# gonewest818/raytrace-clj

Measured on AMD Instinct MI355X. Metric: Msamples/sec (nx*ny*ns), higher is better.
Workload: dtype f64; 1 GPU; C3: 1920x1080x256spp Shirley cover scene n=50 (10001 spheres), depth 50, thin-lens camera, seeded counter RNG; accel=bvh; 8x8 tiles dealt round-robin to 1 GPU(s); nx=1920, ny=1080, ns=256, spheres=10001, depth=50, accel=bvh, accel_ran=bvh, frames_in_flight=1, launch_form=one GPU

## Files before the change

include/rtmi.h:

```cpp
#ifndef RTMI_H
#define RTMI_H

#include <stdint.h>

#ifdef __cplusplus
extern "C" {
#endif

#define RTMI_OK 0
#define RTMI_E_ARG (-1)
#define RTMI_E_DEVICE (-2)
#define RTMI_E_UNSUPPORTED (-3)
#define RTMI_E_NOMEM (-4)
#define RTMI_E_STATE (-5)

enum { RTMI_PRIM_SPHERE = 0, RTMI_PRIM_UVSPHERE = 1, RTMI_PRIM_MOVING = 2,
       RTMI_PRIM_RECT_XY = 3, RTMI_PRIM_RECT_XZ = 4, RTMI_PRIM_RECT_YZ = 5, RTMI_PRIM_TRIANGLE = 6,
       RTMI_PRIM_MEDIUM = 7, RTMI_PRIM_BOUNDARY = 16 };
enum { RTMI_XFORM_TRANSLATE = 0, RTMI_XFORM_ROTATE_Y = 1 };
enum { RTMI_MAT_LAMBERTIAN = 0, RTMI_MAT_METAL = 1, RTMI_MAT_DIELECTRIC = 2, RTMI_MAT_DIFFUSE_LIGHT = 3,
       RTMI_MAT_ISOTROPIC = 4  };
enum { RTMI_TEX_CONSTANT = 0, RTMI_TEX_UVGRADIENT = 1, RTMI_TEX_CHECKER = 2,
       RTMI_TEX_PERLIN_NOISE = 3, RTMI_TEX_PERLIN_TURB = 4, RTMI_TEX_MARBLE = 5, RTMI_TEX_FLIP_U = 6, RTMI_TEX_FLIP_V = 7,
       RTMI_TEX_IMAGE = 8 };
// ... 162 lines not shown
uint64_t rtmi_sample_key(uint64_t seed, uint64_t pixel, uint64_t sample);
int rtmi_probe_arith(rtmi_ctx *ctx, int32_t n, const double *abc, double *out);
#define RTMI_PROBE_MATH_SLOTS 12
int rtmi_probe_math2(rtmi_ctx *ctx, int32_t n, const double *abc, double tmin, double tmax, int32_t n_slots, double *out);
int rtmi_probe_math(rtmi_ctx *ctx, int32_t n, const double *abc, double tmin, double tmax, double *out);

int rtmi_test_build_tree(int32_t n, const double *geom, const double *cam, int32_t threads, uint64_t *out_hash, int32_t *out_info, double *out_ms);
int rtmi_test_camera_fixed(int32_t cam_kind, const double *cam);
int rtmi_test_half_outward(double x, int32_t up);
int rtmi_test_pack_materials(int32_t n_prims, const int32_t *prim_kind, const double *prim_geom, const int32_t *prim_mat,
                             int32_t n_mats, const int32_t *mat_kind, const int32_t *mat_tex, const double *mat_param,
                             int32_t n_tex, const int32_t *tex_kind, const double *tex_param, const int32_t *tex_child,
                             int32_t cam_kind, const double *cam, const int32_t *prim_flip, const int32_t *prim_xform,
                             int32_t n_xforms, const int32_t *xform_kind, const double *xform_param, int32_t through_creation,
                             uint64_t *out_hash, int32_t *out_facts);
int rtmi_test_pack_geometry(int32_t n_prims, const int32_t *prim_kind, const double *prim_geom, const int32_t *prim_mat,
                            int32_t n_mats, const int32_t *mat_kind, const int32_t *mat_tex, const double *mat_param,
                            int32_t n_tex, const int32_t *tex_kind, const double *tex_param, const int32_t *tex_child,
                            int32_t cam_kind, const double *cam, const int32_t *prim_flip, const int32_t *prim_xform,
                            int32_t n_xforms, const int32_t *xform_kind, const double *xform_param, int32_t through_creation, uint64_t *out_hash);
int rtmi_test_refit(int32_t n_prims, const int32_t *prim_kind, const int32_t *prim_flip, const int32_t *prim_xform, int32_t n_xforms, const int32_t *xform_kind,
                    int32_t cam_kind, const double *cam, int32_t n_steps, const double *geoms, const double *xforms,
                    void *out_nodes, int64_t capacity, int64_t *out_bytes, int32_t *out_info, int32_t *out_big,
                    int32_t *out_cells, int64_t cells_capacity, void *out_leaf_box);
int rtmi_test_refit_half(double x, int32_t up);
int rtmi_test_scene_nodes(rtmi_scene *scene, void *buf, int64_t capacity, int64_t *out_bytes);

#ifdef __cplusplus
}
#endif
// ... 2 lines not shown
```

raytrace_clj_amd/_ffi.py:

```python
import ctypes as C
import os

import numpy as np

try:
    import torch
except ImportError:
    torch = None

_HERE = os.path.dirname(os.path.abspath(__file__))
LIB_PATH = os.environ.get("RTMI_LIB") or os.path.join(_HERE, "lib", "librtmi.so")

SYMBOLS = [
    "rtmi_last_error", "rtmi_backend_name", "rtmi_version", "rtmi_init", "rtmi_shutdown", "rtmi_set_option",
    "rtmi_device_info", "rtmi_scene_create", "rtmi_scene_create_ex", "rtmi_scene_set_perlin", "rtmi_scene_set_images", "rtmi_scene_set_media_calls", "rtmi_scene_set_media_mode", "rtmi_scene_set_media_calls_narrowed", "rtmi_scene_device_bytes", "rtmi_scene_destroy", "rtmi_render", "rtmi_render_device",
    "rtmi_render_tiles_device", "rtmi_local_tiles", "rtmi_assemble_device", "rtmi_last_trace_ms", "rtmi_last_reduce_ms", "rtmi_probe_hit",
    "rtmi_probe_paths", "rtmi_probe_camera", "rtmi_probe_texture", "rtmi_probe_scatter", "rtmi_probe_rng",
    "rtmi_sample_key", "rtmi_test_half_outward", "rtmi_test_camera_fixed", "rtmi_test_build_tree", "rtmi_probe_arith", "rtmi_probe_math", "rtmi_probe_math2", "rtmi_last_traversal_counters",
    "rtmi_scene_clone", "rtmi_render_multi", "rtmi_render_multi_device", "rtmi_last_gather_ms",
    "rtmi_last_gather_path", "rtmi_rccl_probe", "rtmi_stream_idle", "rtmi_last_passes", "rtmi_last_accel",
    "rtmi_render_progressive", "rtmi_render_progressive_device", "rtmi_progressive_samples", "rtmi_progressive_release",
    "rtmi_render_adaptive", "rtmi_render_adaptive_device", "rtmi_adaptive_status", "rtmi_adaptive_active_tiles",
    "rtmi_render_features", "rtmi_render_features_device", "rtmi_denoise", "rtmi_denoise_device",
    "rtmi_adaptive_retire", "rtmi_adaptive_retire_device",
    "rtmi_render_adaptive_tiles_device", "rtmi_assemble_progressive_device", "rtmi_render_multi_adaptive", "rtmi_render_multi_adaptive_device",
    "rtmi_scene_set_camera", "rtmi_scene_set_camera_stream", "rtmi_scene_camera",
    "rtmi_reproject", "rtmi_reproject_device",
    "rtmi_scene_tree_info",
    "rtmi_scene_set_materials", "rtmi_scene_set_materials_stream", "rtmi_test_pack_materials",
    "rtmi_scene_set_geometry", "rtmi_scene_last_refit_ms", "rtmi_test_pack_geometry", "rtmi_test_refit", "rtmi_test_refit_half", "rtmi_test_scene_nodes",
]

F64, F32 = 0, 1
ACCEL_FLAT, ACCEL_BVH = 0, 1
FLAG_TIMING = 1
GATHER_PATHS = {0: "none", 1: "same-device", 2: "peer-copy", 3: "rccl"}
SEG_REC = 12
TILE = 8
PROG_REC = 5
FEATURES = 8
EDIT_STREAM_MAX_BYTES = 32768


class RtmiError(RuntimeError):
# ... 75 lines not shown
    L.rtmi_render_features.argtypes =[vp, i32, i32, i32, u64, i32, i32, i32, i32, i32, vp, vp]
    L.rtmi_render_features_device.argtypes = [vp, i32, i32, i32, u64, i32, vp, vp, vp]
    L.rtmi_denoise.argtypes = [vp, i32, i32, vp, vp, vp, i32, dbl, dbl, dbl, dbl, vp, vp, vp]
    L.rtmi_denoise_device.argtypes = [vp, i32, i32, vp, vp, vp, i32, dbl, dbl, dbl, dbl, vp, vp, vp, vp]
    L.rtmi_render_adaptive_tiles_device.argtypes = [vp, i32, i32, i32, i32, i32, dbl, i32, u64, i32, i32, i32, vp, vp, vp]
    L.rtmi_assemble_progressive_device.argtypes = [vp, i32, i32, i32, i32, vp, vp, vp, vp, vp, vp]
    L.rtmi_render_multi_adaptive.argtypes = [i32, C.POINTER(vp), i32, i32, i32, i32, i32, dbl, i32, u64, i32, vp, vp, vp, vp, vp]
    L.rtmi_render_multi_adaptive_device.argtypes = [i32, C.POINTER(vp), i32, i32, i32, i32, i32, dbl, i32, u64, i32, vp, vp, vp, vp, vp]
    L.rtmi_scene_set_camera.argtypes = [vp, i32, vp, C.POINTER(i32)]
    L.rtmi_scene_set_camera_stream.argtypes = [vp, i32, vp, vp]
    L.rtmi_scene_camera.argtypes = [vp, C.POINTER(i32), vp, C.POINTER(dbl), C.POINTER(dbl)]
    L.rtmi_scene_tree_info.argtypes = [vp, vp]
    L.rtmi_scene_set_materials.argtypes = [vp, i32, vp, vp, vp, i32, vp, vp, vp, vp, C.POINTER(i32)]
    L.rtmi_scene_set_materials_stream.argtypes = [vp, i32, vp, vp, vp, i32, vp, vp, vp, vp, vp]
    L.rtmi_test_pack_materials.argtypes = [i32, vp, vp, vp, i32, vp, vp, vp, i32, vp, vp, vp, i32, vp, vp, vp, i32, vp, vp, i32, vp, vp]
    L.rtmi_scene_set_geometry.argtypes = [vp, i32, vp, i32, vp, i32, vp]
    L.rtmi_scene_last_refit_ms.argtypes = [vp, C.POINTER(dbl)]
    L.rtmi_test_pack_geometry.argtypes = [i32, vp, vp, vp, i32, vp, vp, vp, i32, vp, vp, vp, i32, vp, vp, vp, i32, vp, vp, i32, vp]
    L.rtmi_test_refit.argtypes = [i32, vp, vp, vp, i32, vp, i32, vp, i32, vp, vp, vp, i64, vp, vp, vp, vp, i64, vp]
    L.rtmi_test_refit_half.argtypes = [C.c_double, i32]
    L.rtmi_test_scene_nodes.argtypes = [vp, vp, i64, C.POINTER(i64)]
    L.rtmi_reproject.argtypes = [vp, i32, i32, i32, vp, i32, vp] + [vp] * 7 + [dbl] * 5 + [vp] * 5
    L.rtmi_reproject_device.argtypes = [vp, i32, i32, i32, vp, i32, vp] + [vp] * 7 + [dbl] * 5 + [vp] * 6
    for name in SYMBOLS:
        fn = getattr(L, name)
        if fn.restype is C.c_int and name not in ("rtmi_version",):
            fn.restype = C.c_int
    _lib = L
    return L

# ... 17 lines not shown
```

raytrace_clj_amd/csrc/rtmi.hip:

```cpp
#include <hip/hip_runtime.h>
#include <rccl/rccl.h>
#include <dlfcn.h>

#include <algorithm>
#include <atomic>
#include <chrono>
#include <condition_variable>
#include <functional>
#include <thread>
#include <cmath>
#include <cmath>
#include <cstdarg>
#include <cstdio>
#include <cstdlib>
#include <cstring>
#include <array>
#include <map>
#include <mutex>
#include <new>
#include <string>
#include <vector>

#include "rtmi.h"
#include "rtmi_device.h"
// ... 34 lines not shown
    int s_begin, s_count;
    void *samples;
    u64 *counters;
    int prims_per_tile;
    int n_ptiles;
    unsigned *queue;
    unsigned total_items;
    unsigned qblock;
    int suspend_lanes;
    int rx0, ry0, rx1, ry1;
    u64 *trav;
    int susp_off;
    int stash_off;
    double rnx, rny;
    int fixed_rays;
};
#ifndef RTMI_QUEUE_BLOCK
#define RTMI_QUEUE_BLOCK 256
#endif
#ifndef RTMI_EXT_NO_STASH
#define RTMI_EXT_NO_STASH 0
#endif
#ifndef RTMI_EXT_LDS_STASH
#define RTMI_EXT_LDS_STASH 1
#endif
#ifndef RTMI_STASH
#define RTMI_STASH 1
#endif
constexpr unsigned kQueueBlock = RTMI_QUEUE_BLOCK;

// ... 359 lines not shown
            }
            w_cur += min((unsigned)__popcll(dead), avail);
        }
        if (MULTI) { if (!__syncthreads_or(alive ? 1 : 0)) break; }
        else { if (!__any(alive ? 1 : 0)) break; }
        RTMI_PH(PH_REFILL_DEAL)

        R best_t; int best_i;
        intersect_world<R, MULTI, VARIANT, EXT, COUNT, SLICED, MSEQ, !SLICED>(sc, lds, tp.prims_per_tile, tp.n_ptiles, P, alive, tmin, tmax, best_t, best_i, ntrav,
                                                                     &mid, exhausted ? 0 : tp.suspend_lanes, (EXT || LST) ? tp.susp_off : RTMI_BVH_STACK * RTMI_BVH_STRIDE);
        RTMI_PH(PH_BVH_POST)
        if (!SLICED || __any(alive && !mid)) {
        if (alive) {
            if (!mid) ++nrays;
            R emit[3];
            const bool scat = shade_segment<R, EXT>(sc, P, best_t, best_i, nullptr, emit, mid);
            if (!mid && !scat) {
                R *out = reinterpret_cast<R *>(tp.samples) + (size_t)out_item * 3;
                out[0] = emit[0]; out[1] = emit[1]; out[2] = emit[2];
                alive = false;
                RTMI_PH(PH_STORE)
            }
        }
        }
        RTMI_PH(PH_STORE)
    }
    RTMI_STAMP_FLUSH(tp.counters)
    unsigned n = nrays;
    for (int off = 32; off > 0; off >>= 1) n += __shfl_down(n, off);
    if (lane == 0 && n) atomicAdd(tp.counters, (u64)n);
    if (COUNT) {
// ... 798 lines not shown
    int fail_next_render = 0;
    int fail_allocs = 0;
    int last_accel = -1;
    int last_passes = 0;
    int last_grid = 0;
    std::map<std::pair<const void *, size_t>, int> occupancy;
    std::vector<int> tile_ids_host;
    int tile_key[8] = {-1, -1, -1, -1, -1, -1, -1, -1};
    std::vector<hipEvent_t> events_r;
    double last_reduce_ms = 0.0;
    int last_reduce_launches = 0;
    int count_traversal = 0;
    int flat_below = 24;
    bool suspend_lanes_set = false;
    int suspend_lanes = 8;
    hipStream_t last_stream = nullptr;
    long long tile_valid_pixels = 0;
    ProgFrame prog;
    DevBuf feat_out, feat_cnt;
    DevBuf dn_planes, dn_io;
    DevBuf rp_io;
    std::vector<std::pair<hipEvent_t, hipEvent_t>> events;
    int events_used = 0;
};

struct rtmi_scene {
    uint32_t magic = 0x52545343u;
    rtmi_ctx *ctx = nullptr;
    DevScene dev{};
    ScenePtr d_dev = nullptr;
// ... 416 lines not shown
    const TracePlan plan = choose_trace_kernel<R>(s, c, read_launch_knobs(), nptiles > 1, lds_bytes);
    c->last_accel = plan.accel;

    TraceParams tp;
    tp.nx = nx; tp.ny = ny; tp.depth = depth; tp.seed = seed; tp.tiles_x = tiles_x_of(nx);
    tp.n_local_tiles = n_local;
    tp.tile_ids = ad ? reinterpret_cast<const int *>(prog->act_tiles[prog->cur].p) : reinterpret_cast<const int *>(c->tile_ids.p);
    tp.samples = c->samples.p;
    tp.counters = d_counters ? reinterpret_cast<u64 *>(d_counters) : reinterpret_cast<u64 *>(c->counters.p);
    tp.prims_per_tile = (c->scan_variant >= SCAN_SGPR || s->dev.has_ext) ? 0 : ppt; tp.n_ptiles = nptiles;
    tp.queue = reinterpret_cast<unsigned *>(reinterpret_cast<u64 *>(c->counters.p) + 2);
    tp.rx0 = region.x0; tp.ry0 = region.y0; tp.rx1 = region.x1; tp.ry1 = region.y1;
    tp.trav = reinterpret_cast<u64 *>(c->counters.p) + 3;
    tp.suspend_lanes = plan.suspend_lanes; tp.susp_off = plan.lds.susp_off; tp.stash_off = plan.lds.stash_off;
    tp.rnx = 1.0 / (double)nx; tp.rny = 1.0 / (double)ny; tp.fixed_rays = camera_fixed_rays(s->dev.cam_kind, s->dev.cam_fixed_origin, s->dev.cam);
    for (int s_begin = s_first; s_begin < s_end; s_begin += s_per_pass) {
        hipEvent_t e1 = nullptr;
        rc = launch_trace_pass(s, plan, tp, s_begin, std::min(s_per_pass, s_end - s_begin), st, &e1);
        if (!rc) rc = launch_fold<R>(c, tp, ns, s_end, d_tiles_linear, d_counters != nullptr, prog, ad, e1, st);
        if (rc) return rc;
    }
#ifdef RTMI_STAMPS
    rc = report_phase_stamps(c, st);
#endif
    if (!rc && ad)
        HIP_TRY(launch_compact(*prog, nullptr, n_local, -1, tiles_x_of(nx), region, st));
    if (!rc && prog) prog->k = s_end;
    return rc;
}

// ... 69 lines not shown
    auto mix = [&](const void *p, size_t bytes) { const unsigned char *q = (const unsigned char *)p; for (size_t k = 0; k < bytes; ++k) { h ^= q[k]; h *= 1099511628211ull; } };
    mix(nodes.data(), nodes.size() * sizeof(float));
    mix(grid_cells.data(), grid_cells.size() * sizeof(int));
    mix(&d.bvh_root, sizeof(int)); mix(&d.grid_tall, sizeof(int)); mix(&d.bvh_node16, sizeof(int));
    *out_hash = h;
    out_info[0] = (int32_t)(nodes.size() / (d.bvh_node16 ? 8 : 16)); out_info[1] = depth; out_info[2] = d.grid_n; out_info[3] = d.n_big;
    return RTMI_OK;
}
RTMI_EXPORT int rtmi_test_camera_fixed(int32_t cam_kind, const double *cam) {
    const int o = camera_fixed_origin(cam_kind, cam);
    return o | (camera_fixed_rays(cam_kind, o, cam) << 1);
}
RTMI_EXPORT int rtmi_test_half_outward(double x, int32_t up) { return (int)half_outward((float)x, up != 0); }
RTMI_EXPORT const char *rtmi_last_error(void) { return g_err.c_str(); }
RTMI_EXPORT const char *rtmi_backend_name(void) { return "hip-gfx950"; }
RTMI_EXPORT int rtmi_version(void) { return 214; }
RTMI_EXPORT uint64_t rtmi_sample_key(uint64_t seed, uint64_t pixel, uint64_t sample) { return sample_key(seed, pixel, sample); }

RTMI_EXPORT int rtmi_init(int device, uint32_t flags, rtmi_ctx **out_ctx) {
    if (!out_ctx) return fail(RTMI_E_ARG, "out_ctx is NULL");
    *out_ctx = nullptr;
    int ndev = 0;
    if (hipGetDeviceCount(&ndev) != hipSuccess || ndev <= 0) return fail(RTMI_E_DEVICE, "no HIP device visible (this library has no CPU fallback)");
    if (device < 0 || device >= ndev) return fail(RTMI_E_ARG, "device %d out of range (0..%d)", device, ndev - 1);
    HIP_TRY(hipSetDevice(device));
    hipDeviceProp_t prop;
    HIP_TRY(hipGetDeviceProperties(&prop, device));
    if (std::strncmp(prop.gcnArchName, "gfx950", 6) != 0)
        return fail(RTMI_E_DEVICE, "device %d is %s; this library carries gfx950 (MI355X) code objects only", device, prop.gcnArchName);
    rtmi_ctx *c = new (std::nothrow) rtmi_ctx();
    if (!c) return fail(RTMI_E_NOMEM, "out of host memory");
// ... 32 lines not shown
}

RTMI_EXPORT int rtmi_set_option(rtmi_ctx *c, const char *name, int64_t value) {
    if (!ctx_ok(c)) return fail(RTMI_E_STATE, "invalid context handle");
    if (!name) return fail(RTMI_E_ARG, "name is NULL");
    if (!std::strcmp(name, "blocks_per_cu")) { if (value < 1 || value > 64) return fail(RTMI_E_ARG, "blocks_per_cu must be 1..64"); c->blocks_per_cu = (int)value; return RTMI_OK; }
    if (!std::strcmp(name, "workspace_bytes")) { if (value < (1 << 20)) return fail(RTMI_E_ARG, "workspace_bytes must be >= 1 MiB"); c->workspace_bytes = value; return RTMI_OK; }
    if (!std::strcmp(name, "lds_tile_bytes")) { if (value < 1024 || value > 64 * 1024 - 64) return fail(RTMI_E_ARG, "lds_tile_bytes out of range"); c->max_lds_bytes = (int)value; return RTMI_OK; }
    if (!std::strcmp(name, "timing")) { if (value) c->flags |= RTMI_FLAG_TIMING; else c->flags &= ~RTMI_FLAG_TIMING; return RTMI_OK; }
    if (!std::strcmp(name, "scan_variant")) { if (value < 0 || value > 3) return fail(RTMI_E_ARG, "scan_variant must be 0..3"); c->scan_variant = (int)value; return RTMI_OK; }
    if (!std::strcmp(name, "count_traversal")) { c->count_traversal = value ? 1 : 0; return RTMI_OK; }
    if (!std::strcmp(name, "test_fail_next_render")) { c->fail_next_render = value ? 1 : 0; return RTMI_OK; }
    if (!std::strcmp(name, "test_fail_allocs")) { c->fail_allocs = (int)std::max<int64_t>(0, std::min<int64_t>(value, 64)); return RTMI_OK; }
    if (!std::strcmp(name, "flat_below")) { if (value < 0 || value > (1 << 20)) return fail(RTMI_E_ARG, "flat_below must be 0..2^20"); c->flat_below = (int)value; return RTMI_OK; }
    if (!std::strcmp(name, "suspend_lanes")) { if (value < 0 || value > 64) return fail(RTMI_E_ARG, "suspend_lanes must be 0..64"); c->suspend_lanes = (int)value; c->suspend_lanes_set = true; return RTMI_OK; }
    if (!std::strcmp(name, "accel")) {
        if (value == RTMI_ACCEL_FLAT || value == RTMI_ACCEL_BVH) { c->accel = (int)value; return RTMI_OK; }
        return fail(RTMI_E_UNSUPPORTED, "accel %lld is not available in this build", (long long)value);
    }
    return fail(RTMI_E_ARG, "unknown option '%s'", name);
}

RTMI_EXPORT int rtmi_device_info(rtmi_ctx *c, int32_t *cus, int32_t *lds, int64_t *hbm, char *arch, int32_t arch_len) {
    if (!ctx_ok(c)) return fail(RTMI_E_STATE, "invalid context handle");
    if (cus) *cus = c->cus;
    if (lds) *lds = c->lds_per_cu;
    if (hbm) *hbm = (int64_t)c->hbm;
    if (arch && arch_len > 0) { std::strncpy(arch, c->arch.c_str(), (size_t)arch_len - 1); arch[arch_len - 1] = 0; }
    return RTMI_OK;
}
// ... 559 lines not shown
        int rc = check_material_arrays(n_mats, mat_kind, mat_tex, mat_param, n_tex, tex_kind, tex_param, tex_child);
        if (!rc && (n_prims < 0 || (n_prims > 0 && (!prim_kind || !prim_mat)))) rc = fail(RTMI_E_ARG, "primitive arrays are NULL");
        if (!rc) rc = check_material_edit(a);
        if (rc) return rc;
        M = pack_materials(a);
    }
    uint64_t h = 1469598103934665603ull;
    DevScene none{};
    for (const MatTable &t : material_tables(M, none)) {
        const unsigned char *q = (const unsigned char *)t.host;
        for (size_t k = 0; k < t.bytes; ++k) { h ^= q[k]; h *= 1099511628211ull; }
        h ^= (uint64_t)t.bytes; h *= 1099511628211ull;
    }
    *out_hash = h;
    out_facts[0] = M.has_ext ? 1 : 0; out_facts[1] = M.uses_perlin ? 1 : 0; out_facts[2] = M.max_image;
    return RTMI_OK;
}

namespace {
__host__ __device__ inline int refit_key32(unsigned u) { const int v = (int)u; return v ^ ((v >> 31) & 0x7fffffff); }
__host__ __device__ inline int refit_key16(unsigned h) { const int v = (int)(short)(unsigned short)h; return v ^ ((v >> 31) & 0x7fff); }
__host__ __device__ inline unsigned refit_half_outward(unsigned u, bool up) {
    const unsigned sign = u >> 31, a = u & 0x7fffffffu;
    if (a > 0x7f800000u) return 0x7e00u | (sign << 15);
    const bool away = up != (sign != 0);
    unsigned m;
    bool inexact;
    if (a >= 0x47800000u) { m = a == 0x7f800000u ? 0x7c00u : 0x7bffu; inexact = a != 0x7f800000u; }
    else if (a >= 0x38800000u) { m = (((a >> 23) - 112u) << 10) | ((a & 0x7fffffu) >> 13); inexact = (a & 0x1fffu) != 0; }
    else {
// ... 1881 lines not shown
```

raytrace_clj_amd/csrc/rtmi_device.h:

```cpp
#pragma once
#include <hip/hip_runtime.h>
#include <stdint.h>

#include "rtmi.h"

namespace rtmi {

typedef unsigned long long u64;

struct DevScene {
    int n_static;
    int n_moving;
    const double *stat_geom;
    const double *stat4_d;
    const float *stat4_f;
    int n_all;
    const float *cull20;
    const double *exact12;
    double cull_t_lo, cull_t_hi;
    const float *bvh_nodes;
    int bvh_root;
    int n_big;
    int big_idx[16];
    int bvh_node16;
// ... 482 lines not shown

template <typename R> __device__ inline int sin_sign(R x) {
    const R s = Real<R>::sin_(x);
    return s < R(0) ? -1 : (s > R(0) ? 1 : 0);
}
template <> __device__ inline int sin_sign<double>(double x) {
    if (x == 0.0) return 0;
    if (!(fabs(x) <= 1.0e5)) { const double s = ::sin(x); return s < 0.0 ? -1 : (s > 0.0 ? 1 : 0); }
    const double k = ::rint(x * 0.3183098861837907);
    double r = ::fma(-k, 3.141592653589793, x);
    r = ::fma(-k, 1.2246467991473532e-16, r);
    const bool odd = ((int)k) & 1;
    return (odd != (r < 0.0)) ? -1 : 1;
}

template <typename R> __device__ inline R perlin_noise(SceneRef sc, R px, R py, R pz) {
    const R fi = (R)::floor((double)px), fj = (R)::floor((double)py), fk = (R)::floor((double)pz);
    const int i = (int)fi, j = (int)fj, k = (int)fk;
    const R u = px - fi, v = py - fj, w = pz - fk;
    const R uu = (u * u) * (R(3.0) - R(2.0) * u), vv = (v * v) * (R(3.0) - R(2.0) * v), ww = (w * w) * (R(3.0) - R(2.0) * w);
    R acc = R(0);
#pragma unroll
    for (int c = 0; c < 8; ++c) {
        const int di = c >> 2, dj = (c >> 1) & 1, dk = c & 1;
        const int idx = sc.perlin_perm[(i + di) & 255] ^ sc.perlin_perm[256 + ((j + dj) & 255)] ^ sc.perlin_perm[512 + ((k + dk) & 255)];
        const double *g = sc.perlin_vec + (size_t)idx * 3;
        const R A = di ? uu : R(1.0) - uu, B = dj ? vv : R(1.0) - vv, C = dk ? ww : R(1.0) - ww;
        const R d = dot3(u - (R)di, v - (R)dj, w - (R)dk, (R)g[0], (R)g[1], (R)g[2]);
        const R term = ((A * B) * C) * d;
        acc = c ? acc + term : term;
// ... 1162 lines not shown
            if (!ok) {
                t = (-b + sq) / a2;
                ok = (t > tmin) && ((t < best_t) || (t == best_t && orig < best_orig));
            }
            if (ok) { best_t = t; best_i = sc.n_static + m; best_orig = orig; }
        }
    }
}

struct SegLog { double *rec; int max_seg; int n; };

template <typename R> struct HitRec { R t, px, py, pz, nx, ny, nz, u, v; int orig, kind, mat; };

#define RTMI_TEX_CHECKER2 100
#define RTMI_TEX_GRADIENT_REC 101
struct __attribute__((aligned(16))) MatRec { int mat_kind, tex, tex_kind, pad; double param, r, g, b; double scale, c1r, c1g, c1b; double inv_ri, r0; };

#define RTMI_PRIM_NEEDS_U 32
#define RTMI_PRIM_NEEDS_V 64
#define RTMI_PRIM_NEEDS_UV (RTMI_PRIM_NEEDS_U | RTMI_PRIM_NEEDS_V)
template <typename R> __device__ inline void resolve_hit(SceneRef sc, const Path<R> &P, R t, int orig, HitRec<R> &h, bool all_uv = true) {
    const double *g = sc.exact12 + (size_t)orig * 12;
    R cx = (R)g[0], cy = (R)g[1], cz = (R)g[2];
    h.orig = orig;
    const int2 km = reinterpret_cast<const int2 *>(sc.prim_km)[orig];
    if ((km.x & 15) == RTMI_PRIM_MOVING) {
        const R t0 = (R)g[7], t1 = (R)g[8];
        const R f = (P.time - t0) / (t1 - t0), omf = R(1.0) - f;
        cx = (R)g[0] * omf + (R)g[4] * f; cy = (R)g[1] * omf + (R)g[5] * f; cz = (R)g[2] * omf + (R)g[6] * f;
    }
    const int kind_flags = km.x;
// ... 108 lines not shown
    for (int k = info.w - 1; k >= 0; --k) {
        const double *q = sc.ext_xf + (size_t)(info.z + k) * 4;
        if (q[0] == 0.0) { px = px + q[1]; py = py + q[2]; pz = pz + q[3]; }
        else {
            const double sn = q[1], cs = q[2];
            const double rx = cs * px + sn * pz, rz = (-(sn * px)) + cs * pz;
            const double mx = cs * nx + sn * nz, mz = (-(sn * nx)) + cs * nz;
            px = rx; pz = rz; nx = mx; nz = mz;
        }
    }
    h.px = px; h.py = py; h.pz = pz; h.nx = nx; h.ny = ny; h.nz = nz;
}
template <typename R, bool EXT> __device__ inline void resolve_any(SceneRef sc, const Path<R> &P, R t, int orig, HitRec<R> &h, bool all_uv = true) { resolve_hit<R>(sc, P, t, orig, h, all_uv); }
template <> __device__ inline void resolve_any<double, true>(SceneRef sc, const Path<double> &P, double t, int orig, HitRec<double> &h, bool all_uv) { resolve_hit_ext(sc, P, t, orig, h, all_uv); }

template <typename R, bool F4 = false> __device__ inline bool scatter_emit(SceneRef sc, Path<R> &P, const HitRec<R> &h, R *att, R *emit, bool passenger = false) {
    const int mat = h.mat;
    const double2 *mq = reinterpret_cast<const double2 *>(sc.mat_rec + (size_t)mat * 12);
    const double2 m0 = mq[0], m1 = mq[1], m2 = mq[2];
    const int mk = (int)__double2loint(m0.x), mtex = (int)__double2hiint(m0.x), mtk = (int)__double2loint(m0.y);
    const R mparam = (R)m1.x;
    const R px = h.px, py = h.py, pz = h.pz, nx = h.nx, ny = h.ny, nz = h.nz;
    const bool is_light = !passenger && mk == RTMI_MAT_DIFFUSE_LIGHT;
    const bool live = !passenger && !is_light && P.depth > 0;
    const bool is_lamb = live && mk == RTMI_MAT_LAMBERTIAN, is_metal = live && mk == RTMI_MAT_METAL, is_diel = live && mk == RTMI_MAT_DIELECTRIC;
    const bool is_iso = F4 && live && mk == RTMI_MAT_ISOTROPIC;
    bool scat = false;
    emit[0] = emit[1] = emit[2] = R(0);
    R sdx = R(0), sdy = R(0), sdz = R(0);
    R atr = R(1), atg = R(1), atb = R(1);

    R dmag = R(0), ux = P.dx, uy = P.dy, uz = P.dz;
    if (is_metal || is_diel) {
        dmag = Real<R>::sqrt_(dot3(ux, uy, uz, ux, uy, uz));
        if (dmag > R(0)) { const R inv = R(1.0) / dmag; ux = ux * inv; uy = uy * inv; uz = uz * inv; }
// ... 12 lines not shown
        sdx = rx; sdy = ry; sdz = rz;
        P.time = h.t;
        scat = true;
        RTMI_PH(PH_DIRS)
    } else if (is_metal) {
        const R fuzz = mparam;
        const R k = R(2.0) * dot3(ux, uy, uz, nx, ny, nz);
        const R rfx = ux - k * nx, rfy = uy - k * ny, rfz = uz - k * nz;
        sdx = rfx + fuzz * rx; sdy = rfy + fuzz * ry; sdz = rfz + fuzz * rz;
        scat = dot3(sdx, sdy, sdz, nx, ny, nz) > R(0);
        RTMI_PH(PH_DIRS)
    } else if (is_diel) {
        const R ri = mparam;
        const R dn = dot3(P.dx, P.dy, P.dz, nx, ny, nz);
        R onx, ony, onz, eta, cosine;
        if (dn > R(0)) { onx = -nx; ony = -ny; onz = -nz; eta = ri; cosine = ri * (dn / dmag); }
        else { onx = nx; ony = ny; onz = nz; eta = sizeof(R) == sizeof(double) ? (R)mq[5].x : R(1.0) / ri; cosine = -(dn / dmag); }
        const R dt = dot3(ux, uy, uz, onx, ony, onz);
        const R disc = R(1.0) - (eta * eta) * (R(1.0) - dt * dt);
        const R k = R(2.0) * dn;
        sdx = P.dx - k * nx; sdy = P.dy - k * ny; sdz = P.dz - k * nz;
        if (disc > R(0)) {
            R r0;
            if (sizeof(R) == sizeof(double)) r0 = (R)mq[5].y;
            else { r0 = (R(1.0) - ri) / (R(1.0) + ri); r0 = r0 * r0; }
            const R prob = r0 + (R(1.0) - r0) * pow5(R(1.0) - cosine);
            if (!(next_uniform(P) < prob)) {
                const R sq = Real<R>::sqrt_(disc);
                sdx = eta * (ux - onx * dt) - onx * sq;
                sdy = eta * (uy - ony * dt) - ony * sq;
                sdz = eta * (uz - onz * dt) - onz * sq;
            }
// ... 10 lines not shown
        if (n_turb > 0 && n_turb <= RTMI_TURB_WAVE_MAX) {
            double p1 = 0.0;
            if (want_turb) { const double *tp = sc.tex_param + (size_t)mtex * RTMI_TEX_STRIDE; turb_p0 = tp[0]; p1 = tp[1]; }
            const double s = mtk == RTMI_TEX_PERLIN_TURB ? turb_p0 : 1.0;
            turb = perlin_turbulence_wave(sc, want_turb, s * (double)px, s * (double)py, s * (double)pz, (int)p1);
            turb_done = want_turb;
        }
    }
    if (want_tex) {
        R tr, tg, tb;
        if (mtk == RTMI_TEX_CONSTANT) { tr = (R)m1.y; tg = (R)m2.x; tb = (R)m2.y; }
        else if (F4 && turb_done) {
            if (mtk == RTMI_TEX_PERLIN_TURB) tr = tg = tb = R(0.5) * ((R)turb + R(1.0));
            else tr = tg = tb = R(0.5) * (Real<R>::sin_((R)turb_p0 * pz + R(10.0) * (R)turb) + R(1.0));
        }
        else if (mtk == RTMI_TEX_CHECKER2) {
            const double2 m3 = mq[3], m4 = mq[4];
            const R scale = (R)m3.x;
            const int sx = sin_sign<R>(scale * px), sy = sin_sign<R>(scale * py), sz = sin_sign<R>(scale * pz);
            const bool neg = sx * sy * sz < 0;
            tr = neg ? (R)m1.y : (R)m3.y; tg = neg ? (R)m2.x : (R)m4.x; tb = neg ? (R)m2.y : (R)m4.y;
        } else if (mtk == RTMI_TEX_GRADIENT_REC) {
            const double2 *gq = reinterpret_cast<const double2 *>(sc.mat_grad + (size_t)mat * 12);
            const double2 g0 = gq[0], g1 = gq[1], g2 = gq[2], g3 = gq[3], g4 = gq[4], g5 = gq[5];
            const R u = h.u, v = h.v, omu = R(1.0) - u, omv = R(1.0) - v;
            const R a0 = (R)g1.y * omu + (R)g0.x * u, a1 = (R)g2.x * omu + (R)g0.y * u, a2 = (R)g2.y * omu + (R)g1.x * u;
            const R b0 = (R)g4.y * omu + (R)g3.x * u, b1 = (R)g5.x * omu + (R)g3.y * u, b2 = (R)g5.y * omu + (R)g4.x * u;
            tr = b0 * omv + a0 * v; tg = b1 * omv + a1 * v; tb = b2 * omv + a2 * v;
        } else tex_sample<R, F4>(sc, mtex, h.u, h.v, px, py, pz, tr, tg, tb);
        if (is_light) { emit[0] = R(0) + P.ar * tr; emit[1] = R(0) + P.ag * tg; emit[2] = R(0) + P.ab * tb; }
        else { atr = tr; atg = tg; atb = tb; }
        RTMI_PH(PH_TEXTURE)
    }
    if (!scat) return false;
    if (att) { att[0] = atr; att[1] = atg; att[2] = atb; }
    P.ox = px; P.oy = py; P.oz = pz; P.dx = sdx; P.dy = sdy; P.dz = sdz;
    P.ar = P.ar * atr; P.ag = P.ag * atg; P.ab = P.ab * atb;
    P.depth -= 1;
    return true;
}

template <typename R, bool EXT = false>
__device__ inline bool shade_segment(SceneRef sc, Path<R> &P, R t, int orig, SegLog *lg, R *emit, bool passenger = false) {
    emit[0] = emit[1] = emit[2] = R(0);
    if (!passenger && orig < 0) return false;
    HitRec<R> h;
    h.px = h.py = h.pz = h.nx = h.ny = h.nz = h.u = h.v = h.t = R(0); h.mat = 0; h.orig = 0; h.kind = 0;
    if (!passenger) {
        resolve_any<R, EXT>(sc, P, t, orig, h, false);
        RTMI_PH(PH_HITREC)
    }
    const bool scat = scatter_emit<R, EXT>(sc, P, h, nullptr, emit, passenger);
    if (lg && lg->n < lg->max_seg) {
        double *q = lg->rec + (size_t)lg->n * RTMI_SEG_REC;
        q[0] = h.orig; q[1] = h.t; q[2] = h.px; q[3] = h.py; q[4] = h.pz; q[5] = h.nx; q[6] = h.ny; q[7] = h.nz;
        q[8] = scat ? P.dx : 0; q[9] = scat ? P.dy : 0; q[10] = scat ? P.dz : 0; q[11] = scat ? 1.0 : 0.0;
        lg->n++;
    }
    return scat;
}

}
```

raytrace_clj_amd/csrc/scene_build.h:

```cpp
#pragma once
#include <unistd.h>

namespace {

struct BuildKnobs {
    int sah_levels = 1 << 20;
    int sweep_max = 0;
    double min_frac = 0.0;
    bool grid_off = false;
    int grid_side = 0;
    int grid_kmax = 4;
    bool grid_walk = true;
    bool mloc = false;
    int node16 = -1;
    bool box_leaf = false;
    bool small_scan = true;
    bool debug = false;
};
inline BuildKnobs read_build_knobs() {
    BuildKnobs k;
    if (const char *e = std::getenv("RTMI_BVH_SAH_LEVELS")) k.sah_levels = std::atoi(e);
    if (const char *e = std::getenv("RTMI_BVH_SWEEP_MAX")) k.sweep_max = std::atoi(e);
    if (const char *e = std::getenv("RTMI_BVH_MIN_FRAC")) k.min_frac = std::atof(e);
    if (const char *e = std::getenv("RTMI_GRID")) { k.grid_off = e[0] == '0'; k.grid_side = std::atoi(e); }
// ... 634 lines not shown
    bool fixed = cam_kind == RTMI_CAM_PINHOLE || cam[21] == 0.0;
    for (int k = 0; k < 3; ++k) fixed = fixed && camera_component_plain(cam[k]);
    for (int k = 12; k < 18; ++k) fixed = fixed && std::isfinite(cam[k]) && std::isfinite((float)cam[k]);
    return fixed ? 1 : 0;
}
inline int camera_fixed_rays(int cam_kind, int fixed_origin, const double *cam) {
    bool fixed = cam_kind == RTMI_CAM_THINLENS && fixed_origin;
    for (int k = 3; k < 6; ++k) fixed = fixed && camera_component_plain(cam[k]);
    return fixed ? 1 : 0;
}
inline void camera_shutter(int cam_kind, const double *cam, double &t_lo, double &t_hi) {
    t_lo = cam_kind == RTMI_CAM_THINLENS ? std::min(cam[22], cam[23]) : 0.0;
    t_hi = cam_kind == RTMI_CAM_THINLENS ? std::max(cam[22], cam[23]) : 0.0;
}

PackedMaterials pack_materials(const SceneArrays &a) {
    PackedMaterials M;
    const int n_prims = a.n_prims;
    for (int t = 0; t < a.n_tex; ++t) {
        if (a.tex_kind[t] > RTMI_TEX_CHECKER) M.has_ext = true;
        if (a.tex_kind[t] >= RTMI_TEX_PERLIN_NOISE && a.tex_kind[t] <= RTMI_TEX_MARBLE) M.uses_perlin = true;
        if (a.tex_kind[t] == RTMI_TEX_IMAGE) M.max_image = std::max(M.max_image, (int)a.tex_param[(size_t)t * RTMI_TEX_STRIDE]);
    }
    for (int i = 0; i < n_prims; ++i)
        if (a.mat_kind[a.prim_mat[i]] == RTMI_MAT_ISOTROPIC) M.has_ext = true;
    const std::vector<char> uses = texture_uv_use(a);
    M.prim_mat.assign(a.prim_mat, a.prim_mat + n_prims);
    M.prim_kind.resize((size_t)n_prims);
    for (int i = 0; i < n_prims; ++i) {
        const int kind = a.prim_kind[i] & ~RTMI_PRIM_BOUNDARY;
// ... 15 lines not shown
        MatRec r;
        std::memset(&r, 0, sizeof(r));
        r.mat_kind = a.mat_kind[m]; r.tex = a.mat_tex[m]; r.param = a.mat_param[m];
        if (a.mat_kind[m] == RTMI_MAT_DIELECTRIC) {
            const volatile double ri = a.mat_param[m];
            const volatile double inv = 1.0 / ri, num = 1.0 - ri, den = 1.0 + ri;
            const volatile double q = num / den;
            const volatile double r0 = q * q;
            r.inv_ri = inv; r.r0 = r0;
        }
        r.tex_kind = (r.tex >= 0 && r.tex < a.n_tex) ? a.tex_kind[r.tex] : -1;
        if (r.tex_kind == RTMI_TEX_CONSTANT) { const double *tp = a.tex_param + (size_t)r.tex * RTMI_TEX_STRIDE; r.r = tp[0]; r.g = tp[1]; r.b = tp[2]; }
        if (r.tex_kind == RTMI_TEX_UVGRADIENT) {
            std::memcpy(&M.mat_grad[(size_t)m * 12], a.tex_param + (size_t)r.tex * RTMI_TEX_STRIDE, 12 * sizeof(double));
            r.tex_kind = RTMI_TEX_GRADIENT_REC;
        }
        if (r.tex_kind == RTMI_TEX_CHECKER) {
            const int c0 = a.tex_child[2 * (size_t)r.tex], c1 = a.tex_child[2 * (size_t)r.tex + 1];
            if (c0 >= 0 && c0 < a.n_tex && c1 >= 0 && c1 < a.n_tex && a.tex_kind[c0] == RTMI_TEX_CONSTANT && a.tex_kind[c1] == RTMI_TEX_CONSTANT) {
                const double *t0 = a.tex_param + (size_t)c0 * RTMI_TEX_STRIDE, *t1 = a.tex_param + (size_t)c1 * RTMI_TEX_STRIDE;
                r.tex_kind = RTMI_TEX_CHECKER2;
                r.scale = a.tex_param[(size_t)r.tex * RTMI_TEX_STRIDE];
                r.r = t0[0]; r.g = t0[1]; r.b = t0[2]; r.c1r = t1[0]; r.c1g = t1[1]; r.c1b = t1[2];
            }
        }
        static_assert(sizeof(MatRec) == 96, "MatRec is twelve doubles");
        std::memcpy(&M.mat_rec[(size_t)m * 12], &r, sizeof(r));
    }
    M.mat_kind.assign(a.mat_kind, a.mat_kind + a.n_mats); M.mat_tex.assign(a.mat_tex, a.mat_tex + a.n_mats); M.mat_param.assign(a.mat_param, a.mat_param + a.n_mats);
    M.tex_kind.assign(a.tex_kind, a.tex_kind + a.n_tex); M.tex_child.assign(a.tex_child, a.tex_child + 2 * (size_t)a.n_tex);
// ... 218 lines not shown
```

Baseline: 7833 Msamples/s.

## Shortcut u-invariant gradients, straighten checker sign test, single divide in dielectric

Adds a packed fast path for UV-gradient textures whose colours do not vary in u, so they become a one-dimensional lerp in v read from the material record instead of the separate gradient table. Replaces the checker texture's three sin_sign calls with a rint-based range reduction and sign-bit XOR, used when every lane in the wavefront has small coordinates. Computes dn/dmag once in the dielectric scatter. The Shirley cover scene mostly uses constant Lambertian, metal and dielectric materials, so only the dielectric change is likely to run often in this workload.

```diff
diff --git a/include/rtmi.h b/include/rtmi.h
--- a/include/rtmi.h
+++ b/include/rtmi.h
@@ -200,6 +200,8 @@
                              int32_t cam_kind, const double *cam, const int32_t *prim_flip, const int32_t *prim_xform,
                              int32_t n_xforms, const int32_t *xform_kind, const double *xform_param, int32_t through_creation,
                              uint64_t *out_hash, int32_t *out_facts);
+int rtmi_test_material_records(int32_t n_mats, const int32_t *mat_kind, const int32_t *mat_tex, const double *mat_param,
+                               int32_t n_tex, const int32_t *tex_kind, const double *tex_param, const int32_t *tex_child, double *out_records);
 int rtmi_test_pack_geometry(int32_t n_prims, const int32_t *prim_kind, const double *prim_geom, const int32_t *prim_mat,
                             int32_t n_mats, const int32_t *mat_kind, const int32_t *mat_tex, const double *mat_param,
                             int32_t n_tex, const int32_t *tex_kind, const double *tex_param, const int32_t *tex_child,
diff --git a/raytrace_clj_amd/_ffi.py b/raytrace_clj_amd/_ffi.py
--- a/raytrace_clj_amd/_ffi.py
+++ b/raytrace_clj_amd/_ffi.py
@@ -27,7 +27,7 @@
     "rtmi_scene_set_camera", "rtmi_scene_set_camera_stream", "rtmi_scene_camera",
     "rtmi_reproject", "rtmi_reproject_device",
     "rtmi_scene_tree_info",
-    "rtmi_scene_set_materials", "rtmi_scene_set_materials_stream", "rtmi_test_pack_materials",
+    "rtmi_scene_set_materials", "rtmi_scene_set_materials_stream", "rtmi_test_pack_materials", "rtmi_test_material_records",
     "rtmi_scene_set_geometry", "rtmi_scene_last_refit_ms", "rtmi_test_pack_geometry", "rtmi_test_refit", "rtmi_test_refit_half", "rtmi_test_scene_nodes",
 ]
 
@@ -133,6 +133,7 @@
     L.rtmi_scene_set_materials.argtypes = [vp, i32, vp, vp, vp, i32, vp, vp, vp, vp, C.POINTER(i32)]
     L.rtmi_scene_set_materials_stream.argtypes = [vp, i32, vp, vp, vp, i32, vp, vp, vp, vp, vp]
     L.rtmi_test_pack_materials.argtypes = [i32, vp, vp, vp, i32, vp, vp, vp, i32, vp, vp, vp, i32, vp, vp, vp, i32, vp, vp, i32, vp, vp]
+    L.rtmi_test_material_records.argtypes = [i32, vp, vp, vp, i32, vp, vp, vp, vp]
     L.rtmi_scene_set_geometry.argtypes = [vp, i32, vp, i32, vp, i32, vp]
     L.rtmi_scene_last_refit_ms.argtypes = [vp, C.POINTER(dbl)]
     L.rtmi_test_pack_geometry.argtypes = [i32, vp, vp, vp, i32, vp, vp, vp, i32, vp, vp, vp, i32, vp, vp, vp, i32, vp, vp, i32, vp]
diff --git a/raytrace_clj_amd/csrc/rtmi.hip b/raytrace_clj_amd/csrc/rtmi.hip
--- a/raytrace_clj_amd/csrc/rtmi.hip
+++ b/raytrace_clj_amd/csrc/rtmi.hip
@@ -72,6 +72,7 @@
     int stash_off;
     double rnx, rny;
     int fixed_rays;
+    int grad_short;
 };
 #ifndef RTMI_QUEUE_BLOCK
 #define RTMI_QUEUE_BLOCK 256
@@ -461,7 +462,7 @@
         if (alive) {
             if (!mid) ++nrays;
             R emit[3];
-            const bool scat = shade_segment<R, EXT>(sc, P, best_t, best_i, nullptr, emit, mid);
+            const bool scat = shade_segment<R, EXT>(sc, P, best_t, best_i, nullptr, emit, mid, tp.grad_short != 0);
             if (!mid && !scat) {
                 R *out = reinterpret_cast<R *>(tp.samples) + (size_t)out_item * 3;
                 out[0] = emit[0]; out[1] = emit[1]; out[2] = emit[2];
@@ -1290,6 +1291,7 @@
     int flat_below = 24;
     bool suspend_lanes_set = false;
     int suspend_lanes = 8;
+    int gradient_shortcut = 1;
     hipStream_t last_stream = nullptr;
     long long tile_valid_pixels = 0;
     ProgFrame prog;
@@ -1736,6 +1738,7 @@
     tp.trav = reinterpret_cast<u64 *>(c->counters.p) + 3;
     tp.suspend_lanes = plan.suspend_lanes; tp.susp_off = plan.lds.susp_off; tp.stash_off = plan.lds.stash_off;
     tp.rnx = 1.0 / (double)nx; tp.rny = 1.0 / (double)ny; tp.fixed_rays = camera_fixed_rays(s->dev.cam_kind, s->dev.cam_fixed_origin, s->dev.cam);
+    tp.grad_short = c->gradient_shortcut;
     for (int s_begin = s_first; s_begin < s_end; s_begin += s_per_pass) {
         hipEvent_t e1 = nullptr;
         rc = launch_trace_pass(s, plan, tp, s_begin, std::min(s_per_pass, s_end - s_begin), st, &e1);
@@ -1835,7 +1838,7 @@
 RTMI_EXPORT int rtmi_test_half_outward(double x, int32_t up) { return (int)half_outward((float)x, up != 0); }
 RTMI_EXPORT const char *rtmi_last_error(void) { return g_err.c_str(); }
 RTMI_EXPORT const char *rtmi_backend_name(void) { return "hip-gfx950"; }
-RTMI_EXPORT int rtmi_version(void) { return 214; }
+RTMI_EXPORT int rtmi_version(void) { return 215; }
 RTMI_EXPORT uint64_t rtmi_sample_key(uint64_t seed, uint64_t pixel, uint64_t sample) { return sample_key(seed, pixel, sample); }
 
 RTMI_EXPORT int rtmi_init(int device, uint32_t flags, rtmi_ctx **out_ctx) {
@@ -1898,6 +1901,7 @@
     if (!std::strcmp(name, "test_fail_allocs")) { c->fail_allocs = (int)std::max<int64_t>(0, std::min<int64_t>(value, 64)); return RTMI_OK; }
     if (!std::strcmp(name, "flat_below")) { if (value < 0 || value > (1 << 20)) return fail(RTMI_E_ARG, "flat_below must be 0..2^20"); c->flat_below = (int)value; return RTMI_OK; }
     if (!std::strcmp(name, "suspend_lanes")) { if (value < 0 || value > 64) return fail(RTMI_E_ARG, "suspend_lanes must be 0..64"); c->suspend_lanes = (int)value; c->suspend_lanes_set = true; return RTMI_OK; }
+    if (!std::strcmp(name, "gradient_shortcut")) { c->gradient_shortcut = value ? 1 : 0; return RTMI_OK; }
     if (!std::strcmp(name, "accel")) {
         if (value == RTMI_ACCEL_FLAT || value == RTMI_ACCEL_BVH) { c->accel = (int)value; return RTMI_OK; }
         return fail(RTMI_E_UNSUPPORTED, "accel %lld is not available in this build", (long long)value);
@@ -2487,6 +2491,20 @@
     }
     *out_hash = h;
     out_facts[0] = M.has_ext ? 1 : 0; out_facts[1] = M.uses_perlin ? 1 : 0; out_facts[2] = M.max_image;
+    return RTMI_OK;
+}
+
+RTMI_EXPORT int rtmi_test_material_records(int32_t n_mats, const int32_t *mat_kind, const int32_t *mat_tex, const double *mat_param,
+                                           int32_t n_tex, const int32_t *tex_kind, const double *tex_param, const int32_t *tex_child, double *out_records) {
+    if (!out_records) return fail(RTMI_E_ARG, "bad arguments");
+    const int rc = check_material_arrays(n_mats, mat_kind, mat_tex, mat_param, n_tex, tex_kind, tex_param, tex_child);
+    if (rc) return rc;
+    const SceneArrays a{0, nullptr, nullptr, nullptr, n_mats, mat_kind, mat_tex, mat_param, n_tex, tex_kind, tex_param, tex_child,
+                        0, nullptr, nullptr, nullptr, 0, nullptr, nullptr};
+    const int rc2 = check_material_edit(a);
+    if (rc2) return rc2;
+    const PackedMaterials M = pack_materials(a);
+    std::memcpy(out_records, M.mat_rec.data(), (size_t)n_mats * 12 * sizeof(double));
     return RTMI_OK;
 }
 
diff --git a/raytrace_clj_amd/csrc/rtmi_device.h b/raytrace_clj_amd/csrc/rtmi_device.h
--- a/raytrace_clj_amd/csrc/rtmi_device.h
+++ b/raytrace_clj_amd/csrc/rtmi_device.h
@@ -520,6 +520,24 @@
     return (odd != (r < 0.0)) ? -1 : 1;
 }
 
+template <typename R, bool F4 = false> __device__ inline bool checker_neg(R x, R y, R z) {
+#if RTMI_CHECKER_STRAIGHT
+    if constexpr (sizeof(R) == sizeof(double) && !F4) {
+        const bool fast = fabs(x) <= 1.0e5 && fabs(y) <= 1.0e5 && fabs(z) <= 1.0e5;
+        if (!__any(fast ? 0 : 1)) {
+            const double kx = ::rint(x * 0.3183098861837907), ky = ::rint(y * 0.3183098861837907), kz = ::rint(z * 0.3183098861837907);
+            double rx = ::fma(-kx, 3.141592653589793, x), ry = ::fma(-ky, 3.141592653589793, y), rz = ::fma(-kz, 3.141592653589793, z);
+            rx = ::fma(-kx, 1.2246467991473532e-16, rx); ry = ::fma(-ky, 1.2246467991473532e-16, ry); rz = ::fma(-kz, 1.2246467991473532e-16, rz);
+            const unsigned odd = (unsigned)(int)((kx + ky) + kz);
+            const unsigned sgn = (unsigned)(__double2hiint(rx) ^ __double2hiint(ry) ^ __double2hiint(rz));
+            const bool zero = x == 0.0 || y == 0.0 || z == 0.0;
+            return !zero && (((odd << 31) ^ sgn) >> 31) != 0u;
+        }
+    }
+#endif
+    return sin_sign<R>(x) * sin_sign<R>(y) * sin_sign<R>(z) < 0;
+}
+
 template <typename R> __device__ inline R perlin_noise(SceneRef sc, R px, R py, R pz) {
     const R fi = (R)::floor((double)px), fj = (R)::floor((double)py), fk = (R)::floor((double)pz);
     const int i = (int)fi, j = (int)fj, k = (int)fk;
@@ -1712,7 +1730,17 @@
 
 #define RTMI_TEX_CHECKER2 100
 #define RTMI_TEX_GRADIENT_REC 101
-struct __attribute__((aligned(16))) MatRec { int mat_kind, tex, tex_kind, pad; double param, r, g, b; double scale, c1r, c1g, c1b; double inv_ri, r0; };
+#define RTMI_MATREC_GRADIENT_V 1
+#ifndef RTMI_GRADIENT_SHORTCUT
+#define RTMI_GRADIENT_SHORTCUT 1
+#endif
+#ifndef RTMI_CHECKER_STRAIGHT
+#define RTMI_CHECKER_STRAIGHT 1
+#endif
+#ifndef RTMI_DIEL_ONE_DIV
+#define RTMI_DIEL_ONE_DIV 1
+#endif
+struct __attribute__((aligned(16))) MatRec { int mat_kind, tex, tex_kind, tex_flags; double param, r, g, b; double scale, c1r, c1g, c1b; double inv_ri, r0; };
 
 #define RTMI_PRIM_NEEDS_U 32
 #define RTMI_PRIM_NEEDS_V 64
@@ -1851,11 +1879,12 @@
 template <typename R, bool EXT> __device__ inline void resolve_any(SceneRef sc, const Path<R> &P, R t, int orig, HitRec<R> &h, bool all_uv = true) { resolve_hit<R>(sc, P, t, orig, h, all_uv); }
 template <> __device__ inline void resolve_any<double, true>(SceneRef sc, const Path<double> &P, double t, int orig, HitRec<double> &h, bool all_uv) { resolve_hit_ext(sc, P, t, orig, h, all_uv); }
 
-template <typename R, bool F4 = false> __device__ inline bool scatter_emit(SceneRef sc, Path<R> &P, const HitRec<R> &h, R *att, R *emit, bool passenger = false) {
+template <typename R, bool F4 = false> __device__ inline bool scatter_emit(SceneRef sc, Path<R> &P, const HitRec<R> &h, R *att, R *emit, bool passenger = false, bool u_const = false) {
     const int mat = h.mat;
     const double2 *mq = reinterpret_cast<const double2 *>(sc.mat_rec + (size_t)mat * 12);
     const double2 m0 = mq[0], m1 = mq[1], m2 = mq[2];
     const int mk = (int)__double2loint(m0.x), mtex = (int)__double2hiint(m0.x), mtk = (int)__double2loint(m0.y);
+    const bool grad_v = RTMI_GRADIENT_SHORTCUT && sizeof(R) == sizeof(double) && u_const && mtk == RTMI_TEX_GRADIENT_REC && ((int)__double2hiint(m0.y) & RTMI_MATREC_GRADIENT_V);
     const R mparam = (R)m1.x;
     const R px = h.px, py = h.py, pz = h.pz, nx = h.nx, ny = h.ny, nz = h.nz;
     const bool is_light = !passenger && mk == RTMI_MAT_DIFFUSE_LIGHT;
@@ -1898,8 +1927,11 @@
         const R ri = mparam;
         const R dn = dot3(P.dx, P.dy, P.dz, nx, ny, nz);
         R onx, ony, onz, eta, cosine;
-        if (dn > R(0)) { onx = -nx; ony = -ny; onz = -nz; eta = ri; cosine = ri * (dn / dmag); }
-        else { onx = nx; ony = ny; onz = nz; eta = sizeof(R) == sizeof(double) ? (R)mq[5].x : R(1.0) / ri; cosine = -(dn / dmag); }
+        constexpr bool one_div = RTMI_DIEL_ONE_DIV && sizeof(R) == sizeof(double) && !F4;
+        R dq = R(0);
+        if (one_div) dq = dn / dmag;
+        if (dn > R(0)) { onx = -nx; ony = -ny; onz = -nz; eta = ri; cosine = ri * (one_div ? dq : dn / dmag); }
+        else { onx = nx; ony = ny; onz = nz; eta = sizeof(R) == sizeof(double) ? (R)mq[5].x : R(1.0) / ri; cosine = -(one_div ? dq : dn / dmag); }
         const R dt = dot3(ux, uy, uz, onx, ony, onz);
         const R disc = R(1.0) - (eta * eta) * (R(1.0) - dt * dt);
         const R k = R(2.0) * dn;
@@ -1940,12 +1972,16 @@
             if (mtk == RTMI_TEX_PERLIN_TURB) tr = tg = tb = R(0.5) * ((R)turb + R(1.0));
             else tr = tg = tb = R(0.5) * (Real<R>::sin_((R)turb_p0 * pz + R(10.0) * (R)turb) + R(1.0));
         }
-        else if (mtk == RTMI_TEX_CHECKER2) {
+        else if (mtk == RTMI_TEX_CHECKER2 || grad_v) {
             const double2 m3 = mq[3], m4 = mq[4];
-            const R scale = (R)m3.x;
-            const int sx = sin_sign<R>(scale * px), sy = sin_sign<R>(scale * py), sz = sin_sign<R>(scale * pz);
-            const bool neg = sx * sy * sz < 0;
-            tr = neg ? (R)m1.y : (R)m3.y; tg = neg ? (R)m2.x : (R)m4.x; tb = neg ? (R)m2.y : (R)m4.y;
+            if (mtk == RTMI_TEX_CHECKER2) {
+                const R scale = (R)m3.x;
+                const bool neg = checker_neg<R, F4>(scale * px, scale * py, scale * pz);
+                tr = neg ? (R)m1.y : (R)m3.y; tg = neg ? (R)m2.x : (R)m4.x; tb = neg ? (R)m2.y : (R)m4.y;
+            } else {
+                const R v = h.v, omv = R(1.0) - v;
+                tr = (R)m3.y * omv + (R)m1.y * v; tg = (R)m4.x * omv + (R)m2.x * v; tb = (R)m4.y * omv + (R)m2.y * v;
+            }
         } else if (mtk == RTMI_TEX_GRADIENT_REC) {
             const double2 *gq = reinterpret_cast<const double2 *>(sc.mat_grad + (size_t)mat * 12);
             const double2 g0 = gq[0], g1 = gq[1], g2 = gq[2], g3 = gq[3], g4 = gq[4], g5 = gq[5];
@@ -1967,7 +2003,7 @@
 }
 
 template <typename R, bool EXT = false>
-__device__ inline bool shade_segment(SceneRef sc, Path<R> &P, R t, int orig, SegLog *lg, R *emit, bool passenger = false) {
+__device__ inline bool shade_segment(SceneRef sc, Path<R> &P, R t, int orig, SegLog *lg, R *emit, bool passenger = false, bool u_const = false) {
     emit[0] = emit[1] = emit[2] = R(0);
     if (!passenger && orig < 0) return false;
     HitRec<R> h;
@@ -1976,7 +2012,7 @@
         resolve_any<R, EXT>(sc, P, t, orig, h, false);
         RTMI_PH(PH_HITREC)
     }
-    const bool scat = scatter_emit<R, EXT>(sc, P, h, nullptr, emit, passenger);
+    const bool scat = scatter_emit<R, EXT>(sc, P, h, nullptr, emit, passenger, !EXT && u_const);
     if (lg && lg->n < lg->max_seg) {
         double *q = lg->rec + (size_t)lg->n * RTMI_SEG_REC;
         q[0] = h.orig; q[1] = h.t; q[2] = h.px; q[3] = h.py; q[4] = h.pz; q[5] = h.nx; q[6] = h.ny; q[7] = h.nz;
diff --git a/raytrace_clj_amd/csrc/scene_build.h b/raytrace_clj_amd/csrc/scene_build.h
--- a/raytrace_clj_amd/csrc/scene_build.h
+++ b/raytrace_clj_amd/csrc/scene_build.h
@@ -672,6 +672,19 @@
     t_hi = cam_kind == RTMI_CAM_THINLENS ? std::max(cam[22], cam[23]) : 0.0;
 }
 
+inline bool gradient_component_plain(double c) {
+    if (!std::isfinite(c) || !std::isfinite((float)c)) return false;
+    if (c == 0.0) return !std::signbit(c);
+    return std::fabs(c) >= 0x1p-125;
+}
+inline bool gradient_u_invariant(const double *tp) {
+    for (int c = 0; c < 3; ++c) {
+        if (std::memcmp(&tp[c], &tp[3 + c], sizeof(double)) != 0 || std::memcmp(&tp[6 + c], &tp[9 + c], sizeof(double)) != 0) return false;
+        if (!gradient_component_plain(tp[c]) || !gradient_component_plain(tp[6 + c])) return false;
+    }
+    return true;
+}
+
 PackedMaterials pack_materials(const SceneArrays &a) {
     PackedMaterials M;
     const int n_prims = a.n_prims;
@@ -717,6 +730,11 @@
         if (r.tex_kind == RTMI_TEX_UVGRADIENT) {
             std::memcpy(&M.mat_grad[(size_t)m * 12], a.tex_param + (size_t)r.tex * RTMI_TEX_STRIDE, 12 * sizeof(double));
             r.tex_kind = RTMI_TEX_GRADIENT_REC;
+            const double *tp = a.tex_param + (size_t)r.tex * RTMI_TEX_STRIDE;
+            if (gradient_u_invariant(tp)) {
+                r.tex_flags = RTMI_MATREC_GRADIENT_V;
+                r.r = tp[0]; r.g = tp[1]; r.b = tp[2]; r.c1r = tp[6]; r.c1g = tp[7]; r.c1b = tp[8];
+            }
         }
         if (r.tex_kind == RTMI_TEX_CHECKER) {
             const int c0 = a.tex_child[2 * (size_t)r.tex], c1 = a.tex_child[2 * (size_t)r.tex + 1];
```

Result: no change. 7878 Msamples/s (median of 6 runs) (+0.6%).
